# leohuang2013/pyannote-audio_speaker-diarization_cpp

Hardware: AMD Instinct MI355X
Metric: real-time factor (audio-sec/wall-sec), 1 h 16 kHz mono per GPU (higher is better)
Workload: dtype f32

## Files before the change

### pyannote-audio_speaker-diarization_cpp_amd/csrc/api.cpp

```cpp
#include "common.h"
#include "many_plan.h"
#include "wav_file.h"
#include "roster.h"
#include <algorithm>
#include <cmath>
#include <cstdlib>
#include <fstream>
#include <tuple>

static std::string g_create_err;

int seg_prec(const sd_ctx* c) { return c->seg_precision >= 0 ? c->seg_precision : (c->ecapa_precision != 0 ? 3 : 0); }

extern "C" const char* sd_create_error(void) { return g_create_err.c_str(); }
extern "C" const char* sd_last_error(const sd_ctx* c) { return c ? c->err.c_str() : "null context"; }

extern "C" sd_ctx* sd_create(const char* seg_path, const char* emb_path, int device)
{
    g_create_err.clear();
    int ndev = 0;
    if (hipGetDeviceCount(&ndev) != hipSuccess || ndev <= 0) { g_create_err = "no HIP device available (libsdhip has no CPU fallback)"; return nullptr; }
    if (device < 0 || device >= ndev) { g_create_err = "device id out of range"; return nullptr; }
    if (hipSetDevice(device) != hipSuccess) { g_create_err = "hipSetDevice failed"; return nullptr; }
    sd_ctx* c = new sd_ctx();
// ... 51 lines not shown
    }
    c->pending.clear();
}

extern "C" int sd_kernel_stats(const sd_ctx* cc, const char* kernel, double* total_ms, int64_t* launches, double* flops, double* bytes)
{
    sd_ctx* c = const_cast<sd_ctx*>(cc);
    if (!c || !kernel) return SD_ERR_ARG;
    (void)hipStreamSynchronize(c->stream);
    sd_flush_profile(c);
    auto it = c->stats.find(kernel);
    KernelStat s; if (it != c->stats.end()) s = it->second;
    if (total_ms) *total_ms = s.ms; if (launches) *launches = s.launches; if (flops) *flops = s.flops; if (bytes) *bytes = s.bytes;
    return SD_OK;
}
extern "C" int sd_debug_read_ws(sd_ctx* c, const char* name, int64_t offset, void* h_out, int64_t bytes)
{
    if (!c || !name || !h_out || offset < 0 || bytes < 0) return SD_ERR_ARG;
    auto it = c->ws.find(name);
    if (it == c->ws.end() || !it->second.p) SD_FAIL(c, SD_ERR_ARG, "no workspace named %s", name);
    if ((size_t)(offset + bytes) > it->second.cap) SD_FAIL(c, SD_ERR_ARG, "workspace %s holds %zu bytes", name, it->second.cap);
    HIPCHK(c, hipStreamSynchronize(c->stream));
    HIPCHK(c, hipMemcpy(h_out, (const char*)it->second.p + offset, (size_t)bytes, hipMemcpyDeviceToHost));
    return SD_OK;
}
extern "C" void sd_reset_stats(sd_ctx* c) { if (!c) return; (void)hipStreamSynchronize(c->stream); sd_flush_profile(c); c->stats.clear(); }
extern "C" int sd_stage_ms(const sd_ctx* c, double* ms4) { if (!c || !ms4) return SD_ERR_ARG; for (int i = 0; i < 4; ++i) ms4[i] = c->stage_ms[i]; return SD_OK; }
extern "C" int sd_set_option(sd_ctx* c, const char* key, int64_t v)
{
    if (!c || !key) return SD_ERR_ARG;
    std::string k(key);
    if (k == "emb_batch_items") { c->emb_batch_items = v; c->emb_batch_explicit = true; }
    else if (k == "seg_batch_chunks") c->seg_batch_chunks = v;
    else if (k == "ws_limit_mb") g_ws_limit.store(v > 0 ? (size_t)v << 20 : 0);
    else if (k == "emb_batch_default") { c->emb_batch_items = 3072; c->emb_batch_explicit = false; c->embed_calls = v; }
    else if (k == "linkage_wgs") c->linkage_wgs = v;
    else if (k == "linkage_threads") c->linkage_threads = v;
    else if (k == "linkage_kernel") c->linkage_kernel = v;
    else if (k == "linkage_tie_kernel") c->linkage_tie_kernel = v;
    else if (k == "linkage_zero_phase") c->linkage_zero_phase = v;
    else if (k == "linkage_force_heap") c->linkage_force_heap = v != 0;
    else if (k == "linkage_hx_wide") c->linkage_hx_wide = v != 0;
    else if (k == "linkage_prefetch") c->linkage_prefetch = v != 0;
    else if (k == "linkage_one_xcd") c->linkage_one_xcd = v;
    else if (k == "linkage_square") c->linkage_square = v;
    else if (k == "linkage_batch") { if (v != 0 && v != 1) SD_FAIL(c, SD_ERR_ARG, "linkage_batch must be 0 or 1"); c->linkage_batch = v; }
    else if (k == "linkage_batch_bytes") { if (v < 1) SD_FAIL(c, SD_ERR_ARG, "linkage_batch_bytes must be at least 1"); c->linkage_batch_bytes = v; }
    else if (k == "linkage_batch_threads") { if (v != 0 && v != 256 && v != 1024) SD_FAIL(c, SD_ERR_ARG, "linkage_batch_threads must be 0 (auto), 256 or 1024"); c->linkage_batch_threads = v; }
    else if (k == "skip_dead_rows") c->skip_dead_rows = v != 0;
    else if (k == "conv_h256") c->conv_h256 = v != 0;
    else if (k == "conv_glds") c->conv_glds = v != 0;
    else if (k == "conv_pp") c->conv_pp = v != 0;
    else if (k == "conv_glds_f32") c->conv_glds_f32 = v != 0;
    else if (k == "conv_mfma16") { if (v < 0 || v > 2) return SD_ERR_ARG; c->conv_mfma16 = (int)v; }
    else if (k == "conv_rot") { if (v < 0 || v > 3) return SD_ERR_ARG; c->conv_rot = (int)v; }
    else if (k == "conv_stagger") { if (v < 0 || v > 2) return SD_ERR_ARG; c->conv_stagger = (int)v; }
    else if (k == "conv_w256_f32") c->conv_w256_f32 = v != 0;
    else if (k == "conv_pn") c->conv_pn = (int)v;
    else if (k == "ecapa_ld_pad") { if (v < 0 || v > 1024 || ((int64_t)v & 7)) return SD_ERR_ARG; c->ecapa_ld_pad = (int)v; }
    else if (k == "seg_shared_conv0") c->seg_shared_conv0 = v != 0;
    else if (k == "seg_wide_ih") c->seg_wide_ih = v != 0;
    else if (k == "conv_w256_kmin") c->conv_w256_kmin = (int)v;
    else if (k == "conv_pn128") c->conv_pn128 = (int)v;
    else if (k == "seg_precision") { if (v != 0 && v != 3 && v != -1) SD_FAIL(c, SD_ERR_ARG, "seg_precision must be 0 (f32), 3 (split fp16 operands for the LSTM) or -1 (auto: 3 whenever ecapa_precision is not 0)"); c->seg_precision = (int)v; }
    else if (k == "ecapa_precision") { if (v < 0 || v > 3) SD_FAIL(c, SD_ERR_ARG, "ecapa_precision must be 0 (f32), 1 (fp16), 2 (fp16, hi + lo weight planes) or 3 (f32 tensors, split fp16 operands on the wide layers)");
                                        if (hipSetDevice(c->device) != hipSuccess) SD_FAIL(c, SD_ERR_HIP, "hipSetDevice failed");
                                        const int rcw = ensure_ecapa_mode_weights(c, (int)v); if (rcw) return rcw;
                                        c->ecapa_precision = (int)v; }
    else if (k == "ecapa_f16_hp") { if (v != 0 && v != 1 && v != 3) SD_FAIL(c, SD_ERR_ARG, "ecapa_f16_hp must be 0, 1 (MFA output in f32) or 3 (+ the attention branch)"); c->ecapa_f16_hp = (int)v; }
    else if (k == "ecapa_keep_cat") c->ecapa_keep_cat = v != 0;
    else if (k == "rank0_permille") c->rank0_permille = (int)v;
    else if (k == "virtual_world") c->virtual_world = (int)v;
    else if (k == "comm_timeout_ms") c->comm_timeout_ms = v;
    else if (k == "inject_fail_rank") c->inject_fail_rank = (int)v;
    else if (k == "constrained_assignment") c->constrained_assignment = v != 0;
    else if (k == "clustering_method") { if (v < SD_LINKAGE_SINGLE || v > SD_LINKAGE_WEIGHTED) SD_FAIL(c, SD_ERR_ARG, "clustering_method must be one of SD_LINKAGE_SINGLE (0) .. SD_LINKAGE_WEIGHTED (6)"); c->clustering_method = (int)v; }
    else if (k == "min_cluster_size") { if (v < 1 || v > 0x7fffffff) SD_FAIL(c, SD_ERR_ARG, "min_cluster_size must be at least 1"); c->min_cluster_size = (int)v; }
    else if (k == "max_num_embeddings") { if (v != -1 && v < 1) SD_FAIL(c, SD_ERR_ARG, "max_num_embeddings must be -1 (every train row) or at least 1"); c->max_num_embeddings = v; }
    else if (k == "clustering_seed") c->clustering_seed = v;
    else if (k == "num_clusters") c->num_clusters = (int)v;
    else if (k == "min_clusters") c->min_clusters = (int)v;
    else if (k == "max_clusters") c->max_clusters = (int)v;
    else if (k == "activity_hamming") { if (v != 0 && v != 1) SD_FAIL(c, SD_ERR_ARG, "activity_hamming must be 0 or 1"); c->activity_hamming = v != 0; }
    else if (k == "cut_group_bytes") { if (v < 1) SD_FAIL(c, SD_ERR_ARG, "cut_group_bytes must be at least 1"); c->cut_group_bytes = v; }
    else if (k == "profile") { c->profile = v != 0; c->profile_detail = v >= 2; }
    else SD_FAIL(c, SD_ERR_ARG, "unknown option %s", key);
    return SD_OK;
}

extern "C" int sd_set_option_f64(sd_ctx* c, const char* key, double v)
{
    if (!c || !key) return SD_ERR_ARG;
    std::string k(key);
    if (k == "clustering_threshold") { if (!(v >= 0.0 && v <= 2.0)) SD_FAIL(c, SD_ERR_ARG, "clustering_threshold must lie in [0, 2]"); c->clustering_threshold = v; }
    else if (k == "activity_onset") { if (!(v >= 0.0 && v <= 1.0)) SD_FAIL(c, SD_ERR_ARG, "activity_onset must lie in [0, 1]"); c->activity_onset = v; }
    else if (k == "activity_offset") { if (!(v >= 0.0 && v <= 1.0)) SD_FAIL(c, SD_ERR_ARG, "activity_offset must lie in [0, 1]"); c->activity_offset = v; }
    else if (k == "activity_min_duration_on") { if (!(v >= 0.0)) SD_FAIL(c, SD_ERR_ARG, "activity_min_duration_on must be >= 0"); c->activity_min_on = v; }
    else if (k == "activity_min_duration_off") { if (!(v >= 0.0)) SD_FAIL(c, SD_ERR_ARG, "activity_min_duration_off must be >= 0"); c->activity_min_off = v; }
    else if (k == "speaker_match_threshold") { if (!(v >= 0.0 && v <= 2.0)) SD_FAIL(c, SD_ERR_ARG, "speaker_match_threshold must lie in [0, 2]"); c->speaker_match_threshold = v; }
    else SD_FAIL(c, SD_ERR_ARG, "unknown real-valued option %s", key);
    return SD_OK;
}
extern "C" int sd_linkage_method_from_name(const char* name)
{
    static const char* const names[] = {"single", "complete", "average", "centroid", "median", "ward", "weighted"};
    if (!name) return -1;
// ... 462 lines not shown
```

### pyannote-audio_speaker-diarization_cpp_amd/csrc/common.h

```cpp
#pragma once
#include <hip/hip_runtime.h>
#include <atomic>
#include <chrono>
#include <cstdint>
#include <cstdio>
#include <cstring>
#include <map>
#include <set>
#include <string>
#include <functional>
#include <initializer_list>
#include <vector>
#include "../../include/sdhip_test.h"
#include "cluster_host.h"
#include "many_plan.h"

#define SD_T 501
#define SD_TP 501
#define SD_NBINS 201
#define SD_NMELS 80
#define SD_FEAT_LD 96

#define SD_WAV_PAD 512
struct DevWav {
// ... 14 lines not shown
    int reserve(size_t bytes) {
        if (bytes <= cap) return 0;
        const auto t0 = std::chrono::steady_clock::now();
        if (p) (void)hipFree(p);
        const auto t1 = std::chrono::steady_clock::now();
        p = nullptr; cap = 0;
        size_t want = bytes + (bytes >> 3) + 256;
        const size_t lim = g_ws_limit.load(std::memory_order_relaxed);
        if ((lim && bytes > lim) || hipMalloc(&p, want) != hipSuccess) { p = nullptr; (void)hipGetLastError(); return 1; }
        const auto t2 = std::chrono::steady_clock::now();
        g_ws_free_us += (long long)std::chrono::duration<double, std::micro>(t1 - t0).count();
        g_ws_alloc_us += (long long)std::chrono::duration<double, std::micro>(t2 - t1).count();
        g_ws_alloc_bytes += want; ++g_ws_allocs;
        cap = want; return 0;
    }
    void release() { if (p) (void)hipFree(p); p = nullptr; cap = 0; }
    template <class T> T* as() const { return (T*)p; }
};

struct ConvLayer {
    float* W = nullptr;
    void* W16 = nullptr;
    float* bias = nullptr;
    float* scale = nullptr;
    float* shift = nullptr;
    int Cin = 0, CinPad = 0, Cout = 0, KT = 1, dil = 1;
    int CinPad16 = 0;
    void* W16x = nullptr;
    float w16x_inv = 1.0f;
};

struct ConvArgs {
    const float* X; const float* X2; const float* W; float* Y;
    const void* W16;
    const float* bias; const float* scale; const float* shift; const float* item_bias; const float* R;
    int x_ld, x2_ld, y_ld, r_ld, ib_ld;
    int w_ld;
    int M;
    int TpIn, TpOut;
    int Tin, T;
    int Cin, Cout, KT, dil;
    int cin_real;
    int pad_mode;
    int act1, act2;
    int m_tiles, n_tiles;
    int sched;
    const int2* rowtab;
    int in_rows;
    int y_f32;
    int kt_real;
    int prec;
    const void* W16x;
    float acc_scale;
    int stagger;
};
#define ROWTAB_T(y) ((y) & 1023)
#define ROWTAB_LAST(y) (((y) >> 10) & 1023)
#define ROWTAB_ITEM(y) ((int)((unsigned)(y) >> 20))
#define ROWTAB_MAX_ITEMS 4095

struct EcapaWeights {
    bool loaded = false;
    float* mel_w = nullptr; int* mel_lo = nullptr; int* mel_cnt = nullptr; int* mel_off = nullptr; int mel_nnz = 0;
    float* window = nullptr;
    double* tw_cos = nullptr;
    double* tw_nsin = nullptr;
    ConvLayer block0;
    struct SERes { ConvLayer tdnn1, res[7], tdnn2, se1, se2; int dil; } blk[3];
    ConvLayer mfa, asp_tdnn_x, asp_tdnn_ms, asp_conv, fc;
    int C = 1024;
    std::vector<ConvLayer*> conv16;
    bool have16 = false, have16x = false;
};

struct SegWeights {
    bool loaded = false;
    float wn_w = 1, wn_b = 0;
    ConvLayer conv0, conv1, conv2;
    float* conv0_wsum = nullptr;
    float* in_w[3] = {nullptr, nullptr, nullptr};
    float* in_b[3] = {nullptr, nullptr, nullptr};
    ConvLayer lstm_ih[4];
    float* lstm_hh[4][2] = {};
    void* lstm_hh_x[4][2] = {};
    float lstm_hh_inv[4][2] = {};
    ConvLayer lin0, lin1;
    float* cls_w = nullptr; float* cls_b = nullptr;
};

struct StepStash {
    bool clustered = false;
    int64_t N = 0; int K = 0;
    std::vector<int> clusters, cluster_res, hard_pre;
    std::vector<double> X, Xn, soft;
    int64_t ar0 = 0, cr0 = 0, rows = 0, crow_all = 0, nact = 0;
    int64_t infer_items = 0;
};

struct JobResult { std::vector<double> conf, cen; std::vector<int64_t> cen_counts; int cen_K = 0, cen_d = 0; std::vector<int32_t> enrolled, hard, roster_ids; };

struct ManyJob { int status = SD_OK; JobResult res; };

struct sd_ctx {
    int device = 0;
    hipStream_t stream = nullptr;
    std::string err;
    EcapaWeights ew;
    SegWeights sw;
    std::vector<void*> owned;
    char* warena_cur = nullptr; size_t warena_left = 0;
    std::map<std::string, DevBuf> ws;
    std::set<std::string> rs_taps_filled;
    std::map<std::string, KernelStat> stats;
    bool profile = false;
    bool profile_detail = false;
    std::vector<std::tuple<std::string, hipEvent_t, hipEvent_t, double, double>> pending;
    double stage_ms[4] = {0, 0, 0, 0};
    int64_t emb_batch_items = 3072;
    bool emb_batch_explicit = false;
    int64_t embed_calls = 0;
    int64_t seg_batch_chunks = 4096;
    int num_clusters = -1, min_clusters = -1, max_clusters = -1;
    int ecapa_precision = 0;
    int seg_precision = -1;
    bool ecapa_keep_cat = false;
    int ecapa_f16_hp = 0;
    bool conv_w256_f32 = true;
    int conv_pn128 = 0;
    int ecapa_ld_pad = 0;
    bool seg_wide_ih = true;
    bool seg_shared_conv0 = true;
    int conv_w256_kmin = 0;
    int conv_pn = 0;
    bool conv_h256 = true;
    int conv_mfma16 = 1;
    int conv_rot = 3;
    int conv_stagger = 0;
    bool conv_glds_f32 = false;
    bool conv_pp = true;
    bool conv_glds = true;
    bool skip_dead_rows = true;
    int64_t linkage_wgs = -1;
    int64_t linkage_square = -1;
    int64_t linkage_one_xcd = 1;
    int64_t linkage_zero_phase = 1;
    int64_t linkage_tie_kernel = 1;
    int64_t linkage_prefetch = 0;
    bool linkage_hx_wide = false;
    bool linkage_force_heap = false;
    int64_t linkage_kernel = -1;
    int64_t linkage_threads = 0;
    int64_t linkage_batch = 0;
    int64_t linkage_batch_bytes = (int64_t)2 << 30;
    int64_t linkage_batch_threads = 0;
    std::vector<double> ahead_Z; int64_t ahead_N = -1;
    int num_cu = 256;
    bool constrained_assignment = false;
    int clustering_method = SD_LINKAGE_CENTROID;
    double clustering_threshold = (double)0.7153814381597874f;
    int min_cluster_size = 15;
    int64_t max_num_embeddings = -1;
    bool stream_intact = false;
    int64_t clustering_seed = 0;
    JobResult last;
    DevBuf enr_gal, enr_m2;
    std::vector<double> enr_host;
    int64_t enr_M = 0;
    int enr_d = 0;
    double speaker_match_threshold = (double)0.7153814381597874f * (double)0.7153814381597874f / 2;
    double activity_onset = 0.5, activity_offset = 0.5, activity_min_on = 0.0, activity_min_off = 0.0;
    bool activity_hamming = false;
    std::vector<double> last_activity;
    int64_t fe_bill_samples = -1, fe_bill_frames = 0;
    void* comm = nullptr;
    int rank = 0, world = 1;
    int virtual_world = 0;
    int64_t comm_timeout_ms = 600000;
    int64_t job_seq = 0;
    int inject_fail_rank = -1;
    int rank0_permille = -1;
    std::string dump_dir;
    int dump_level = 0;
    StepStash stash;
    std::string ws_failed;
    int fe_last_grid = 0;
    const char* last_conv_kernel = nullptr;
    const float* planted_scores = nullptr;
    const float* planted_emb = nullptr;
    int64_t planted_lo = 0, planted_n = 0;
    std::vector<ManyJob> many_jobs;
// ... 22 lines not shown
#define ENTER(ctx) do { if (!(ctx)) return SD_ERR_ARG; (ctx)->err.clear(); if (hipSetDevice((ctx)->device) != hipSuccess) SD_FAIL(ctx, SD_ERR_HIP, "hipSetDevice failed"); } while (0)
#define GRID1(n) dim3((unsigned)(((n) + 255) / 256)), dim3(256)
inline double now_ms() { return std::chrono::duration<double, std::milli>(std::chrono::steady_clock::now().time_since_epoch()).count(); }

struct ProfScope {
    sd_ctx* c; std::string name; hipEvent_t e0 = nullptr, e1 = nullptr; double flops, bytes;
    ProfScope(sd_ctx* ctx, const std::string& n, double fl = 0, double by = 0) : c(ctx), name(n), flops(fl), bytes(by) {
        if (c->profile) { (void)hipEventCreate(&e0); (void)hipEventCreate(&e1); (void)hipEventRecord(e0, c->stream); }
    }
    ~ProfScope() {
        if (c->profile) { (void)hipEventRecord(e1, c->stream); c->pending.emplace_back(name, e0, e1, flops, bytes); }
        else { KernelStat& s = c->stats[name]; s.launches++; s.flops += flops; s.bytes += bytes; }
    }
};
void sd_flush_profile(sd_ctx* c);

inline int conv_tiles_grid(const sd_ctx* c, ConvArgs& a, int tile_m, int tile_n, int wgs_per_cu)
{
    a.m_tiles = (a.M + tile_m - 1) / tile_m;
    a.n_tiles = (a.Cout + tile_n - 1) / tile_n;
    int g = (wgs_per_cu * c->num_cu / 8) * 8;
    if (g < 8) g = 8;
    const int lx_max = ((a.m_tiles + 7) / 8) * a.n_tiles;
    if (g / 8 > lx_max) g = lx_max * 8;
    return g;
}
struct ConvBill { double flops, bytes; };
inline ConvBill conv_bill(const ConvArgs& a, double rows, bool f16, int inputs = 1)
{
    const int cin = a.cin_real > 0 ? a.cin_real : a.Cin;
    const int kt_alg = a.kt_real > 0 ? a.kt_real : a.KT;
    return {2.0 * rows * a.Cout * cin * kt_alg, (f16 ? 2.0 : 4.0) * (rows * cin * inputs + rows * a.Cout + (double)a.Cout * cin * a.KT)};
}
inline bool conv_set_dyn_lds(const sd_ctx* c, std::atomic<unsigned>& mask, std::initializer_list<const void*> kernels, size_t lds_bytes)
{
    const unsigned dev_bit = 1u << (c->device & 31);
    if (mask.load(std::memory_order_acquire) & dev_bit) return true;
    for (const void* k : kernels)
        if (hipFuncSetAttribute(k, hipFuncAttributeMaxDynamicSharedMemorySize, (int)lds_bytes) != hipSuccess) { (void)hipGetLastError(); return false; }
    mask.fetch_or(dev_bit, std::memory_order_release);
    return true;
}
struct ConvProfWide {
    ProfScope all, prec, wide, caller;
    ConvProfWide(sd_ctx* c, const char* tag, const char* p, const ConvBill& b)
        : all(c, c->profile_detail ? std::string("conv_gemm:") + tag : std::string("conv_gemm"), b.flops, b.bytes),
          prec(c, std::string("conv_gemm_") + p, b.flops, b.bytes), wide(c, std::string("conv_w256_") + p, b.flops, b.bytes),
          caller(c, strcmp(tag, "lstm_ih") == 0 ? "conv_w256_seg" : "conv_w256_ecapa", b.flops, b.bytes) {}
};
int launch_conv_gemm(sd_ctx* c, const ConvArgs& a, const char* tag);
int launch_conv_gemm_h256(sd_ctx* c, const ConvArgs& a, const char* tag);
int launch_conv_gemm_g256(sd_ctx* c, const ConvArgs& a, const char* tag);
int launch_conv_gemm_pp(sd_ctx* c, const ConvArgs& a, const char* tag);
int seg_prec(const sd_ctx* c);
int launch_conv_narrow(sd_ctx* c, const ConvArgs& a, const char* tag);
struct PackTensor { std::vector<int64_t> dims; std::vector<float> data; };
typedef std::map<std::string, PackTensor> Pack;
int load_pack(const char* path, Pack& out, std::string& err);
int load_model_any(const char* path, int kind, Pack& out, std::string& err);
int build_ecapa_weights(sd_ctx* c, const Pack& p);
int build_seg_weights(sd_ctx* c, const Pack& p);
float lstm_whh_split(const float* whh , _Float16* planes );
void* weight_alloc(sd_ctx* c, size_t bytes);
int ensure_ecapa_mode_weights(sd_ctx* c, int ecapa_precision);
inline size_t conv_w16_bytes(const ConvLayer& L) { return (size_t)2 * L.KT * L.Cout * L.CinPad16 * 2; }
inline size_t conv_w16x_bytes(const ConvLayer& L) { return (size_t)2 * L.KT * L.Cout * L.CinPad * 2; }
int build_conv_w16(sd_ctx* c, ConvLayer& L, void* d);
int build_conv_w16x(sd_ctx* c, ConvLayer& L, void* d, unsigned* d_max);
int frontend_prepare(sd_ctx* c, const float* d_masks, int64_t items, int64_t first_item, float* d_wav_lens, int* d_nnorm, int* d_nvalid,
                     int* d_flags, bool compact, int* h_n_active, int* d_cidx, std::vector<int>* h_nvalid = nullptr);
int frontend_features(sd_ctx* c, const DevWav& w, int64_t first_item, int64_t run_items, bool compact, const int* d_nnorm,
                      const int* d_rowoff, float* d_feats , bool sig_mode = false);
int embed_signals_frames(sd_ctx* c, const float* h_wav_lens, int64_t B, std::vector<int>& nv, std::vector<int>& nn);
int frontend_prepare_signals(sd_ctx* c, int64_t items);
#define EC_SPACES 4
struct EcapaRowPlan {
    int64_t n = 0;
    std::vector<int> off[EC_SPACES];
    const int* d_off = nullptr;
};
int ecapa_need_rows(int nvalid, bool skip_dead_rows);
int ecapa_build_rowtab(sd_ctx* c, const int* d_off_out, int base_out, const int* d_off_in, int base_in, int64_t items, int2* d_rowtab);
int ecapa_rows_to_half(sd_ctx* c, const float* d_f32, void* d_f16, int64_t n4);
int ecapa_feats_to_half(sd_ctx* c, const float* d_f32, void* d_f16, int64_t rows);
int ecapa_scatter_emb(sd_ctx* c, const float* d_emb_c, const int* d_cidx, float* d_emb, int64_t items);
int launch_masked_mean(sd_ctx* c, bool f16, const void* x, int ld, const int* nvalid, const int* rowoff, int row_base, int64_t items, int64_t rows, float* out, int C);
int launch_se_apply(sd_ctx* c, bool f16, const void* t2, int t2_ld, const float* gate, const void* res, int res_ld, void* y, int y_ld, int C, int64_t rows,
                    const int2* rowtab, const int2* res_map, const int2* out_map);
int launch_asp_stats(sd_ctx* c, bool f16, const void* x, int ld, const int* nvalid, const int* rowoff, int row_base, int64_t items, int64_t rows, float* ms, int C);
int launch_asp_pool(sd_ctx* c, bool f16, const void* x, const float* logit, int ld, const int* nvalid, const int* rowoff, int row_base, int64_t items, int64_t rows,
                    float* pooled, int C);
int ecapa_row_plan(sd_ctx* c, const int* h_nvalid, int64_t n, EcapaRowPlan& plan, int* d_off );
int run_ecapa(sd_ctx* c, const float* d_feats, const int* d_nvalid , const EcapaRowPlan& plan, int64_t a0, int64_t a1, float* d_emb );
std::vector<int64_t> ecapa_plan_batches(const EcapaRowPlan& plan, int64_t cap_rows, bool balance);
int64_t ecapa_round_items(int64_t nb);
int ecapa_run_items(sd_ctx* c, const float* d_feats, const int* d_nvalid, const EcapaRowPlan& plan, int64_t nb, bool balance, float* d_emb);
int run_embed(sd_ctx* c, const DevWav& w, const float* d_masks, int64_t items, int64_t first_item, float* d_emb);
int run_segment(sd_ctx* c, const DevWav& w, int64_t chunk_lo, int64_t chunk_hi, float* d_seg);
int run_segment_rows(sd_ctx* c, const DevWav& rows, int T, float* d_seg, int* frames);
int launch_chunk_norm(sd_ctx* c, const float* d_wav, int64_t origin, int64_t first_chunk, int64_t hop, int L, int64_t chunks, float w, float b, float* xn);
int launch_chunk_stats(sd_ctx* c, const float* d_wav, int64_t origin, int64_t first_chunk, int L, int64_t chunks, float w, float b, float2* st);
int launch_pool_norm(sd_ctx* c, int stage, const float* in, int64_t chunks, int Lc, const float* gw, const float* gb, float* out,
                     const float2* cst, const float* wsum, int chunk_rows);
int launch_lstm_rec(sd_ctx* c, const float* G, const float* whh_f, const float* whh_b, const void* whx_f, const void* whx_b, float inv_f, float inv_b,
                    float* H, int64_t B, int F);
int launch_classifier(sd_ctx* c, const float* y, const float* W, const float* bias, float* seg, int64_t chunks, int F);
// ... 62 lines not shown
```

### pyannote-audio_speaker-diarization_cpp_amd/csrc/conv_gemm.hip

```cpp
#include "conv_dev.h"
#include <type_traits>

#define BM 128
#define BN 128
#define BK 32
#define LDP 36
#define SD_CONV_SCHED_DEFAULT 3

template <bool HAS_X2, int PR>
__global__ __launch_bounds__(256, 2) void k_conv_gemm(ConvArgs a)
{
    constexpr bool F16 = PR == 1, X3 = PR == 3;
    __shared__ __attribute__((aligned(16))) float As[2][BM * LDP];
    __shared__ __attribute__((aligned(16))) float Bs[2][BN * LDP];

    ConvSched sch;
    int q0;
    if (!sch.init(a, a.sched >= 100 ? a.sched - 100 : 8 , q0)) return;
    const int wl = sch.wl, wpx = sch.wpx;

    const int tid = threadIdx.x;
    const int lane = tid & 63, wid = tid >> 6;
    const int wr = wid >> 1, wc = wid & 1;
    const int c4 = tid & 7, r0 = tid >> 3;
// ... 391 lines not shown
        acc = __builtin_amdgcn_mfma_f32_32x32x2f32(av.x, bv.x, acc, 0, 0, 0);
        acc = __builtin_amdgcn_mfma_f32_32x32x2f32(av.y, bv.y, acc, 0, 0, 0);
        acc = __builtin_amdgcn_mfma_f32_32x32x2f32(av.z, bv.z, acc, 0, 0, 0);
        acc = __builtin_amdgcn_mfma_f32_32x32x2f32(av.w, bv.w, acc, 0, 0, 0);
    }
    if (w > 0) {
#pragma unroll
        for (int r = 0; r < 16; ++r) part[w - 1][r][lane] = acc[r];
    }
    __syncthreads();
    if (w != 0) return;
    const int co = n0 + li;
    const bool col_ok = co < a.Cout;
    const float cb = (a.bias && col_ok) ? a.bias[co] : 0.0f;
    const float cs = (a.scale && col_ok) ? a.scale[co] : 1.0f, ch = (a.scale && col_ok) ? a.shift[co] : 0.0f;
    const float slope = conv_act_slope(a.act1);
#pragma unroll
    for (int r = 0; r < 16; ++r) {
        float v = ((acc[r] + part[0][r][lane]) + part[1][r][lane]) + part[2][r][lane];
        v += cb;
        v = v > 0.0f ? v : v * slope;
        v = v * cs + ch;
        if (a.act2 == 1) v = tanhf(v);
        else if (a.act2 == 2) v = 1.0f / (1.0f + expf(-v));
        const int g = m0 + (r & 3) + 8 * (r >> 2) + 4 * lh;
        if (g < a.M && col_ok) a.Y[(size_t)g * a.y_ld + co] = v;
    }
}

int launch_conv_gemm(sd_ctx* c, const ConvArgs& in, const char* tag)
{
    ConvArgs a = in;
    if (a.w_ld <= 0) a.w_ld = a.Cin;
    const bool f16 = a.prec == 1;
    if (f16 && !a.W16) SD_FAIL(c, SD_ERR_ARG, "conv_gemm(%s): fp16 mode without fp16 weights", tag);
    if (a.Cin % (f16 ? 64 : BK) != 0) SD_FAIL(c, SD_ERR_ARG, "conv_gemm(%s): Cin=%d not a multiple of %d", tag, a.Cin, f16 ? 64 : BK);
    if (a.M <= 0) return SD_OK;
    if (f16 && c->conv_h256 && c->conv_pp) { const int r = launch_conv_gemm_pp(c, a, tag); if (r != 1) return r; }
    if ((f16 && c->conv_h256 && c->conv_glds) || (!f16 && a.prec == 0 && c->conv_w256_f32 && c->conv_glds_f32)) { const int r = launch_conv_gemm_g256(c, a, tag); if (r != 1) return r; }
    if ((f16 && c->conv_h256) || (!f16 && c->conv_w256_f32) || a.prec == 3) { const int r = launch_conv_gemm_h256(c, a, tag); if (r != 1) return r; }
    const bool x3 = a.prec == 3 && a.W16x != nullptr;
    if (a.prec == 3 && !x3) a.prec = 0;
    if (x3) a.w_ld = 2 * a.Cin;
    if (a.prec == 0 && a.KT == 1 && a.M <= SD_SKINNY_MAX_ROWS && a.TpIn == a.M && a.TpOut == a.M && a.T == a.M && a.Tin == a.M && !a.X2 && !a.item_bias && !a.R && !a.rowtab &&
        (a.x_ld & 3) == 0 && (a.w_ld & 3) == 0) {
        const int cinr = a.cin_real > 0 ? a.cin_real : a.Cin;
        ProfScope ps(c, c->profile_detail ? std::string("skinny_gemm:") + tag : std::string("skinny_gemm"), 2.0 * a.M * a.Cout * cinr,
                     4.0 * ((double)a.M * cinr + (double)a.M * a.Cout + (double)a.Cout * cinr));
        c->last_conv_kernel = "skinny";
        hipLaunchKernelGGL(k_skinny_gemm, dim3((a.M + 31) / 32, (a.Cout + 31) / 32), dim3(256), 0, c->stream, a);
        KCHECK(c);
        return SD_OK;
    }
    a.sched = c->conv_pn128 > 0 ? 100 + c->conv_pn128 : SD_CONV_SCHED_DEFAULT;
    a.stagger = c->conv_stagger;
    const int grid = conv_tiles_grid(c, a, BM, BN, 2);
    const double rows = a.rowtab ? (double)a.M
                                 : (double)(a.M / a.TpOut) * a.T + (double)((a.M % a.TpOut) < a.T ? (a.M % a.TpOut) : a.T);
    const ConvBill bill = conv_bill(a, rows, f16, a.X2 ? 2 : 1);
    ProfScope ps(c, c->profile_detail ? std::string("conv_gemm:") + tag : std::string("conv_gemm"), bill.flops, bill.bytes);
    ProfScope ps16(c, f16 ? "conv_gemm_f16" : x3 ? "conv_gemm_x3" : "conv_gemm_f32", bill.flops, bill.bytes);
    c->last_conv_kernel = f16 ? (a.X2 ? "gemm128_f16_x2" : "gemm128_f16") : x3 ? (a.X2 ? "gemm128_x3_x2" : "gemm128_x3") : (a.X2 ? "gemm128_f32_x2" : "gemm128_f32");
    if (f16) {
        if (a.X2) hipLaunchKernelGGL((k_conv_gemm<true, 1>), dim3(grid), dim3(256), 0, c->stream, a);
        else hipLaunchKernelGGL((k_conv_gemm<false, 1>), dim3(grid), dim3(256), 0, c->stream, a);
    } else if (x3) {
        if (a.X2) hipLaunchKernelGGL((k_conv_gemm<true, 3>), dim3(grid), dim3(256), 0, c->stream, a);
        else hipLaunchKernelGGL((k_conv_gemm<false, 3>), dim3(grid), dim3(256), 0, c->stream, a);
    } else if (a.X2) hipLaunchKernelGGL((k_conv_gemm<true, 0>), dim3(grid), dim3(256), 0, c->stream, a);
    else hipLaunchKernelGGL((k_conv_gemm<false, 0>), dim3(grid), dim3(256), 0, c->stream, a);
    KCHECK(c);
    return SD_OK;
}

__global__ void k_fill_rand(float* p, int64_t n, unsigned seed)
{
    int64_t i = (int64_t)blockIdx.x * blockDim.x + threadIdx.x;
    if (i >= n) return;
    unsigned x = (unsigned)i * 2654435761u + seed;
    x ^= x >> 15; x *= 2246822519u; x ^= x >> 13;
    p[i] = ((float)(x & 0xffffff) / 8388608.0f - 1.0f) * 0.5f;
}

extern "C" int sd_bench_conv(sd_ctx* c, int64_t items, int Tp, int T, int Cin, int Cout, int KT, int dil, int has_x2, int dbg, int reps, double* ms_per_launch)
{
    if (!c || !ms_per_launch || items <= 0 || Cin % BK) return SD_ERR_ARG;
    c->err.clear();
    if (hipSetDevice(c->device) != hipSuccess) return SD_ERR_HIP;
    const int64_t M = items * Tp;
    if (dbg < 0 || dbg % 10 != 0) SD_FAIL(c, SD_ERR_ARG, "sd_bench_conv: ablation %d: the ablation builds of k_conv_gemm are retired", dbg % 10);
    const int pad = (dbg / 100) * 32;
    dbg %= 100;
    const int xld = Cin + pad, wld = Cin + pad, yld = Cout + pad;
    WS(c, float, X, "bc_X", M * xld);
    WS(c, float, X2, "bc_X2", has_x2 ? M * xld : 16);
    WS(c, float, W, "bc_W", (int64_t)KT * Cout * wld);
    WS(c, float, Y, "bc_Y", M * yld);
    WS(c, float, B, "bc_B", 3 * Cout);
    hipLaunchKernelGGL(k_fill_rand, dim3((unsigned)((M * xld + 255) / 256)), dim3(256), 0, c->stream, X, M * xld, 1u);
    if (has_x2) hipLaunchKernelGGL(k_fill_rand, dim3((unsigned)((M * xld + 255) / 256)), dim3(256), 0, c->stream, X2, M * xld, 2u);
    hipLaunchKernelGGL(k_fill_rand, dim3((unsigned)(((int64_t)KT * Cout * wld + 255) / 256)), dim3(256), 0, c->stream, W, (int64_t)KT * Cout * wld, 3u);
    hipLaunchKernelGGL(k_fill_rand, dim3((unsigned)((3 * Cout + 255) / 256)), dim3(256), 0, c->stream, B, (int64_t)3 * Cout, 4u);
    ConvArgs a; memset(&a, 0, sizeof(a));
    a.X = X; a.x_ld = xld; a.X2 = has_x2 ? X2 : nullptr; a.x2_ld = xld; a.W = W; a.w_ld = wld; a.Y = Y; a.y_ld = yld;
    a.bias = B; a.scale = B + Cout; a.shift = B + 2 * Cout; a.act1 = 1;
    a.M = (int)M; a.TpIn = a.TpOut = Tp; a.Tin = a.T = T; a.Cin = Cin; a.Cout = Cout; a.KT = KT; a.dil = dil; a.pad_mode = 0;
// ... 17 lines not shown
```

### pyannote-audio_speaker-diarization_cpp_amd/csrc/ecapa.hip

```cpp
#include "common.h"
#include <algorithm>

template <class T> __global__ void k_masked_mean(const T* __restrict__ x, int ld, const int* __restrict__ nvalid, const int* __restrict__ rowoff, int row_base,
                              float* __restrict__ out, int C)
{
    const int item = blockIdx.y, ch = blockIdx.x * blockDim.x + threadIdx.x;
    if (ch >= C) return;
    const int nv = nvalid[item];
    const T* p = x + (size_t)(rowoff[item] - row_base) * ld + ch;
    float s0 = 0, s1 = 0, s2 = 0, s3 = 0;
    int t = 0;
    for (; t + 3 < nv; t += 4) { s0 += (float)p[(size_t)t * ld]; s1 += (float)p[(size_t)(t + 1) * ld]; s2 += (float)p[(size_t)(t + 2) * ld]; s3 += (float)p[(size_t)(t + 3) * ld]; }
    for (; t < nv; ++t) s0 += (float)p[(size_t)t * ld];
    out[(size_t)item * C + ch] = ((s0 + s1) + (s2 + s3)) / (float)nv;
}

template <class T> struct Vec4;
template <> struct Vec4<float> { typedef float4 type; };
template <> struct Vec4<_Float16> { typedef _Float16 type __attribute__((ext_vector_type(4))); };
template <class T> __device__ __forceinline__ float4 ld4(const T* p)
{
    if constexpr (sizeof(T) == 4) return *(const float4*)p;
    else { const typename Vec4<_Float16>::type h = *(const typename Vec4<_Float16>::type*)p; return make_float4((float)h[0], (float)h[1], (float)h[2], (float)h[3]); }
}
// ... 215 lines not shown
    const float* d_feats = d_feats_all + (size_t)rbase[0] * SD_FEAT_LD;
    const int* d_nvalid = d_nvalid_all + a0;
    float* d_emb = d_emb_all + (size_t)a0 * SD_EMB_DIM;
    const int64_t M = R[0], MN = R[3];
    if (M > 0x7fffffff / 2) SD_FAIL(c, SD_ERR_ARG, "ecapa batch too large");
    WS(c, T, x0, "ec_x0", M * LD);
    const int LDT = 2 * C - C / 8 + c->ecapa_ld_pad;
    WS(c, T, tr, "ec_tr", M * LDT);
    WS(c, T, t2, "ec_t2", R[1] * LD);
    WS(c, T, cat, "ec_cat", R[1] * LD3);
    WS(c, T, mfa, "ec_mfa", MN * LD3);
    WS(c, T, hid, "ec_hid", MN * 128);
    WS(c, float, se_s, "ec_se_s", items * C);
    WS(c, float, se_h, "ec_se_h", items * 128);
    WS(c, float, se_g, "ec_se_g", items * C);
    WS(c, float, ms, "ec_ms", items * 2 * C3);
    WS(c, float, ib, "ec_ib", items * 128);
    WS(c, float, pooled, "ec_pooled", items * 2 * C3);
    int rc;
    const bool f16 = sizeof(T) == 2;
    int2* tabs[EC_SPACES][EC_SPACES] = {};
    auto tab = [&](int so, int si) -> int2* {
        if (tabs[so][si]) return tabs[so][si];
        char key[32]; snprintf(key, sizeof(key), "ec_rowtab_%d%d", so, si);
        int2* p = ws_get<int2>(c, key, (size_t)R[so] + 128);
        if (!p) return nullptr;
        if (ecapa_build_rowtab(c, ro[so], rbase[so], ro[si], rbase[si], items, p)) return nullptr;
        tabs[so][si] = p;
        return p;
    };
#define TAB(var, so, si) int2* var = tab(so, si); if (!var) SD_FAIL(c, SD_ERR_HIP, "hipMalloc of a row table failed")

    const void* f_in = d_feats; int f_ld = SD_FEAT_LD;
    if (sizeof(T) == 2) {
        WS(c, _Float16, fh, "ec_feats16", M * 128);
        if ((rc = ecapa_feats_to_half(c, d_feats, fh, M))) return rc;
        f_in = fh; f_ld = 128;
    }
    { TAB(t00, 0, 0); ConvArgs a = conv_args(E.block0, f_in, f_ld, x0, LD, M, true, P); a.act1 = 1; a.rowtab = t00; if ((rc = launch_conv_gemm(c, a, "block0"))) return rc; }

    for (int b = 0; b < 3; ++b) {
        const auto& B = E.blk[b];
        const int cs = b, os = b + 1, is = b == 0 ? 0 : 1;
        const int64_t Mc = R[cs], Mo = R[os];
        const T* xin = (b == 0) ? x0 : cat + (size_t)(b - 1) * C;
        const int xin_ld = (b == 0) ? LD : LD3;
        TAB(t_in, cs, is); TAB(t_cc, cs, cs); TAB(t_oc, os, cs);
        { ConvArgs a = conv_args(B.tdnn1, xin, xin_ld, tr, LDT, Mc, true, P); a.act1 = 1; a.rowtab = t_in; a.in_rows = (int)R[is]; if ((rc = launch_conv_gemm(c, a, "tdnn1"))) return rc; }
        const int S = C / 8;
        for (int i = 1; i < 8; ++i) {
            ConvArgs a = conv_args(B.res[i - 1], tr + (i - 1) * S, LDT, tr + C + (i - 1) * S, LDT, Mc, true, P);
            a.act1 = 1;
            if (i >= 2) { a.X2 = (const float*)(tr + C + (i - 2) * S); a.x2_ld = LDT; }
            a.rowtab = t_cc;
            if ((rc = launch_conv_gemm(c, a, "res2net"))) return rc;
        }
        { ConvArgs a = conv_args(B.tdnn2, tr + C - S, LDT, t2, LD, Mo, true, P); a.act1 = 1; a.rowtab = t_oc; a.in_rows = (int)Mc; if ((rc = launch_conv_gemm(c, a, "tdnn2"))) return rc; }
        if ((rc = launch_masked_mean(c, f16, t2, LD, d_nvalid, ro[os], rbase[os], items, Mo, se_s, C))) return rc;
        { ConvArgs a = conv_args(B.se1, se_s, C, se_h, 128, items, false); a.act1 = 1; if ((rc = launch_conv_gemm(c, a, "se1"))) return rc; }
        { ConvArgs a = conv_args(B.se2, se_h, 128, se_g, C, items, false); a.act2 = 2; if ((rc = launch_conv_gemm(c, a, "se2"))) return rc; }
        {
            const int2* res_map = nullptr; const int2* out_map = nullptr;
            if (os != is) { TAB(m, os, is); res_map = m; }
            if (os != 1) { TAB(m, os, 1); out_map = m; }
            if ((rc = launch_se_apply(c, f16, t2, LD, se_g, xin, xin_ld, cat + (size_t)b * C, LD3, C, Mo, t_oc, res_map, out_map))) return rc;
        }
    }
    TAB(t31, 3, 1); TAB(t33, 3, 3);
    const int hp = sizeof(T) == 2 ? c->ecapa_f16_hp : 0;
    float* mfa32 = nullptr;
    if (hp & 1) { WS(c, float, m32, "ec_mfa32", MN * LD3); mfa32 = m32; }
    {
        ConvArgs a = conv_args(E.mfa, cat, LD3, mfa32 ? (void*)mfa32 : (void*)mfa, LD3, MN, true, P);
        a.act1 = 1; a.rowtab = t31; a.in_rows = (int)R[1]; a.y_f32 = mfa32 ? 1 : 0;
        if ((rc = launch_conv_gemm(c, a, "mfa"))) return rc;
    }
    if (mfa32 && !(hp & 2)) {
        if ((rc = ecapa_rows_to_half(c, mfa32, mfa, MN * LD3 / 4))) return rc;
    }
    const void* pool_x = mfa32 ? (const void*)mfa32 : (const void*)mfa;
    const bool pool_f16 = f16 && !mfa32;
    if ((rc = launch_asp_stats(c, pool_f16, pool_x, LD3, d_nvalid, ro[3], rbase[3], items, MN, ms, C3))) return rc;
    { ConvArgs a = conv_args(E.asp_tdnn_ms, ms, 2 * C3, ib, 128, items, false); if ((rc = launch_conv_gemm(c, a, "asp_ms"))) return rc; }
    float* logits;
    if (sizeof(T) == 2 || c->ecapa_keep_cat) { WS(c, float, lg, "ec_logits", MN * LD3); logits = lg; } else logits = (float*)cat;
    if (hp & 2) {
        WS(c, float, hid32, "ec_hid32", MN * 128);
        { ConvArgs a = conv_args(E.asp_tdnn_x, mfa32, LD3, hid32, 128, MN, true, 0); a.act1 = 1; a.act2 = 1; a.item_bias = ib; a.ib_ld = 128; a.rowtab = t33; if ((rc = launch_conv_gemm(c, a, "asp_tdnn"))) return rc; }
        { ConvArgs a = conv_args(E.asp_conv, hid32, 128, logits, LD3, MN, true, 0); a.rowtab = t33; if ((rc = launch_conv_gemm(c, a, "asp_conv"))) return rc; }
    } else {
        { ConvArgs a = conv_args(E.asp_tdnn_x, mfa, LD3, hid, 128, MN, true, P); a.act1 = 1; a.act2 = 1; a.item_bias = ib; a.ib_ld = 128; a.rowtab = t33; if ((rc = launch_conv_gemm(c, a, "asp_tdnn"))) return rc; }
        { ConvArgs a = conv_args(E.asp_conv, hid, 128, logits, LD3, MN, true, P); a.rowtab = t33; a.y_f32 = 1; if ((rc = launch_conv_gemm(c, a, "asp_conv"))) return rc; }
    }
    if ((rc = launch_asp_pool(c, pool_f16, pool_x, logits, LD3, d_nvalid, ro[3], rbase[3], items, MN, pooled, C3))) return rc;
    { ConvArgs a = conv_args(E.fc, pooled, 2 * C3, d_emb, SD_EMB_DIM, items, false); if ((rc = launch_conv_gemm(c, a, "fc"))) return rc; }
    return SD_OK;
}

__global__ void k_flag_nonfinite(const float* e, int64_t n, int* flag)
{
    const int64_t i = (int64_t)blockIdx.x * blockDim.x + threadIdx.x;
    if (i < n && !isfinite(e[i])) *flag = 1;
}

int run_ecapa(sd_ctx* c, const float* d_feats, const int* d_nvalid, const EcapaRowPlan& plan, int64_t a0, int64_t a1, float* d_emb)
{
    if (c->ecapa_precision == 1 || c->ecapa_precision == 2) return run_ecapa_t<_Float16>(c, d_feats, d_nvalid, plan, a0, a1, d_emb);
// ... 175 lines not shown
```

Baseline: 2968.

## Add persistent panel kernel for f32 Res2Net dilated convolutions

```diff
diff --git a/pyannote-audio_speaker-diarization_cpp_amd/csrc/api.cpp b/pyannote-audio_speaker-diarization_cpp_amd/csrc/api.cpp
--- a/pyannote-audio_speaker-diarization_cpp_amd/csrc/api.cpp
+++ b/pyannote-audio_speaker-diarization_cpp_amd/csrc/api.cpp
@@ -127,6 +127,7 @@
     else if (k == "conv_glds") c->conv_glds = v != 0;
     else if (k == "conv_pp") c->conv_pp = v != 0;
     else if (k == "conv_glds_f32") c->conv_glds_f32 = v != 0;
+    else if (k == "conv_res2_panel") c->conv_res2_panel = v != 0;
     else if (k == "conv_mfma16") { if (v < 0 || v > 2) return SD_ERR_ARG; c->conv_mfma16 = (int)v; }
     else if (k == "conv_rot") { if (v < 0 || v > 3) return SD_ERR_ARG; c->conv_rot = (int)v; }
     else if (k == "conv_stagger") { if (v < 0 || v > 2) return SD_ERR_ARG; c->conv_stagger = (int)v; }
diff --git a/pyannote-audio_speaker-diarization_cpp_amd/csrc/common.h b/pyannote-audio_speaker-diarization_cpp_amd/csrc/common.h
--- a/pyannote-audio_speaker-diarization_cpp_amd/csrc/common.h
+++ b/pyannote-audio_speaker-diarization_cpp_amd/csrc/common.h
@@ -90,6 +90,7 @@
     int prec;
     const void* W16x;
     float acc_scale;
+    int same_space;
     int stagger;
 };
 #define ROWTAB_T(y) ((y) & 1023)
@@ -174,6 +175,7 @@
     int conv_mfma16 = 1;
     int conv_rot = 3;
     int conv_stagger = 0;
+    bool conv_res2_panel = true;
     bool conv_glds_f32 = false;
     bool conv_pp = true;
     bool conv_glds = true;
@@ -302,6 +304,7 @@
 int launch_conv_gemm_h256(sd_ctx* c, const ConvArgs& a, const char* tag);
 int launch_conv_gemm_g256(sd_ctx* c, const ConvArgs& a, const char* tag);
 int launch_conv_gemm_pp(sd_ctx* c, const ConvArgs& a, const char* tag);
+int launch_conv_res2_panel(sd_ctx* c, const ConvArgs& a, const char* tag);
 int seg_prec(const sd_ctx* c);
 int launch_conv_narrow(sd_ctx* c, const ConvArgs& a, const char* tag);
 struct PackTensor { std::vector<int64_t> dims; std::vector<float> data; };
diff --git a/pyannote-audio_speaker-diarization_cpp_amd/csrc/conv_gemm.hip b/pyannote-audio_speaker-diarization_cpp_amd/csrc/conv_gemm.hip
--- a/pyannote-audio_speaker-diarization_cpp_amd/csrc/conv_gemm.hip
+++ b/pyannote-audio_speaker-diarization_cpp_amd/csrc/conv_gemm.hip
@@ -467,6 +467,7 @@
         KCHECK(c);
         return SD_OK;
     }
+    { const int r = launch_conv_res2_panel(c, a, tag); if (r != 1) return r; }
     a.sched = c->conv_pn128 > 0 ? 100 + c->conv_pn128 : SD_CONV_SCHED_DEFAULT;
     a.stagger = c->conv_stagger;
     const int grid = conv_tiles_grid(c, a, BM, BN, 2);
diff --git a/pyannote-audio_speaker-diarization_cpp_amd/csrc/conv_res2.hip b/pyannote-audio_speaker-diarization_cpp_amd/csrc/conv_res2.hip
--- /dev/null
+++ b/pyannote-audio_speaker-diarization_cpp_amd/csrc/conv_res2.hip
@@ -0,0 +1,191 @@
+#include "conv_dev.h"
+
+#define RP_BM 128
+#define RP_HALO 4
+#define RP_ROWS (RP_BM + 2 * RP_HALO)
+#define RP_LD 132
+#define RP_WLD 36
+#define RP_PARTS ((RP_ROWS * 32 + 511) / 512)
+#define RP_LDS_BYTES ((RP_ROWS * RP_LD + 2 * 128 * RP_WLD) * 4)
+
+static std::atomic<unsigned> g_attr_res2{0};
+
+template <bool HAS_X2>
+__global__ __launch_bounds__(512, 1) void k_conv_res2_panel(ConvArgs a)
+{
+    extern __shared__ __attribute__((aligned(16))) float lds[];
+    float* const Ps = lds;
+    float* const Ws = lds + RP_ROWS * RP_LD;
+
+    const int G = gridDim.x;
+    int tile = blockIdx.x;
+    if (tile >= a.m_tiles) return;
+    const int tid = threadIdx.x, lane = tid & 63, wid = tid >> 6;
+    const int wr = wid >> 1, wc = wid & 1, li = lane & 31, lh = lane >> 5;
+    const int d = a.dil;
+    const int in_rows = a.M;
+    const int prow = tid >> 5, pch = tid & 31;
+    const int wrow = tid >> 3, wch = tid & 7;
+
+    auto panel_rsrc = [&](const float* X, int ld, int m0, bool live) {
+        int lo = m0 - d; if (lo < 0) lo = 0;
+        int hi = m0 + RP_BM + d; if (hi > in_rows) hi = in_rows;
+        const int rows = live && hi > lo ? hi - lo : 0;
+        return conv_rsrc(X + (live ? (size_t)lo * ld : 0), (size_t)rows * ld * 4);
+    };
+    const unsigned voA0 = (unsigned)(prow * a.x_ld + pch * 4) * 4u, stA = (unsigned)a.x_ld * 64u;
+    const unsigned voX0 = HAS_X2 ? (unsigned)(prow * a.x2_ld + pch * 4) * 4u : 0u, stX = HAS_X2 ? (unsigned)a.x2_ld * 64u : 0u;
+    f4u pa[RP_PARTS], px[2];
+    auto pstore = [&]() {
+#pragma unroll
+        for (int p = 0; p < RP_PARTS; ++p)
+            if (prow + 16 * p < RP_ROWS) *(float4*)&Ps[(prow + 16 * p) * RP_LD + pch * 4] = make_float4(pa[p][0], pa[p][1], pa[p][2], pa[p][3]);
+    };
+
+    const __amdgpu_buffer_rsrc_t rB = conv_rsrc(a.W, (size_t)3 * 128 * a.w_ld * 4);
+    const unsigned voB0 = (unsigned)(wrow * a.w_ld + wch * 4) * 4u, stB = (unsigned)a.w_ld * 256u;
+    f4u rb[2];
+    auto wload = [&](int s) {
+        const unsigned so = (unsigned)((s >> 2) * 128 * a.w_ld + (s & 3) * 32) * 4u;
+        rb[0] = __builtin_bit_cast(f4u, __builtin_amdgcn_raw_buffer_load_b128(rB, voB0, so, 0));
+        rb[1] = __builtin_bit_cast(f4u, __builtin_amdgcn_raw_buffer_load_b128(rB, voB0 + stB, so, 0));
+    };
+    auto wstore = [&](int buf) {
+#pragma unroll
+        for (int p = 0; p < 2; ++p) *(float4*)&Ws[buf * 128 * RP_WLD + (wrow + 64 * p) * RP_WLD + wch * 4] = make_float4(rb[p][0], rb[p][1], rb[p][2], rb[p][3]);
+    };
+
+    int poff[3];
+    auto set_rows = [&](int2 e, int m0) {
+        const int t = ROWTAB_T(e.y), last = ROWTAB_LAST(e.y);
+#pragma unroll
+        for (int kk = 0; kk < 3; ++kk) {
+            int pr = e.x + conv_src_frame(t, kk, 3, 1, d, a.Tin, last) - (m0 - d);
+            pr = pr < 0 ? 0 : (pr > RP_ROWS - 1 ? RP_ROWS - 1 : pr);
+            poff[kk] = pr * RP_LD + lh * 16;
+        }
+    };
+    auto tab_entry = [&](int m0) { const int g = m0 + wr * 32 + li; return a.rowtab[g < a.M ? g : a.M - 1]; };
+
+    f32x16 acc[2];
+#pragma unroll
+    for (int j = 0; j < 2; ++j)
+#pragma unroll
+        for (int r = 0; r < 16; ++r) acc[j][r] = 0.0f;
+    const int boff = (wc * 64 + li) * RP_WLD + lh * 16;
+    float4 fa[2], fb[2][2];
+    auto lfrag = [&](int s, int qq, int set) {
+        const float* Ab = Ps + poff[s >> 2] + (s & 3) * 32 + qq * 4;
+        const float* Bb = Ws + (s & 1) * 128 * RP_WLD + boff + qq * 4;
+        fa[set] = *(const float4*)Ab;
+        fb[set][0] = *(const float4*)Bb;
+        fb[set][1] = *(const float4*)(Bb + 32 * RP_WLD);
+    };
+    auto mma8 = [&](int set) {
+        const float av[4] = {fa[set].x, fa[set].y, fa[set].z, fa[set].w};
+        const float bv0[4] = {fb[set][0].x, fb[set][0].y, fb[set][0].z, fb[set][0].w}, bv1[4] = {fb[set][1].x, fb[set][1].y, fb[set][1].z, fb[set][1].w};
+#pragma unroll
+        for (int e = 0; e < 4; ++e) {
+            acc[0] = __builtin_amdgcn_mfma_f32_32x32x2f32(av[e], bv0[e], acc[0], 0, 0, 0);
+            acc[1] = __builtin_amdgcn_mfma_f32_32x32x2f32(av[e], bv1[e], acc[1], 0, 0, 0);
+        }
+    };
+
+    int m0 = tile * RP_BM;
+    {
+        const int shift = m0 < d ? d - m0 : 0;
+        const __amdgpu_buffer_rsrc_t rA = panel_rsrc(a.X, a.x_ld, m0, true), rX = panel_rsrc(HAS_X2 ? a.X2 : a.X, HAS_X2 ? a.x2_ld : a.x_ld, m0, true);
+#pragma unroll
+        for (int p = 0; p < RP_PARTS; ++p) {
+            const bool ok = prow + 16 * p >= shift;
+            pa[p] = __builtin_bit_cast(f4u, __builtin_amdgcn_raw_buffer_load_b128(rA, ok ? voA0 + p * stA - (unsigned)shift * a.x_ld * 4u : 0x80000000u, 0, 0));
+            if (HAS_X2) pa[p] += __builtin_bit_cast(f4u, __builtin_amdgcn_raw_buffer_load_b128(rX, ok ? voX0 + p * stX - (unsigned)shift * a.x2_ld * 4u : 0x80000000u, 0, 0));
+        }
+        wload(0);
+        set_rows(tab_entry(m0), m0);
+        pstore();
+        wstore(0);
+    }
+    __syncthreads();
+    lfrag(0, 0, 0);
+
+    const float slope = conv_act_slope(a.act1);
+    const unsigned ybytes = (unsigned)a.y_ld * 4u;
+    float cb_[2], cs_[2], ch_[2];
+#pragma unroll
+    for (int j = 0; j < 2; ++j) conv_col_params(a, wc * 64 + j * 32 + li, cb_[j], cs_[j], ch_[j]);
+
+    while (true) {
+        const int ntile = tile + G;
+        const bool has_next = ntile < a.m_tiles;
+        const int m0n = ntile * RP_BM;
+        const __amdgpu_buffer_rsrc_t rA = panel_rsrc(a.X, a.x_ld, m0n, has_next), rX = panel_rsrc(HAS_X2 ? a.X2 : a.X, HAS_X2 ? a.x2_ld : a.x_ld, m0n, has_next);
+        const int2 en = tab_entry(has_next ? m0n : m0);
+
+#pragma unroll
+        for (int s = 0; s < 12; ++s) {
+            lfrag(s, 1, 1);
+            wload((s + 1) % 12);
+            if (s < RP_PARTS) {
+                pa[s] = __builtin_bit_cast(f4u, __builtin_amdgcn_raw_buffer_load_b128(rA, voA0 + s * stA, 0, 0));
+                if (HAS_X2) px[s & 1] = __builtin_bit_cast(f4u, __builtin_amdgcn_raw_buffer_load_b128(rX, voX0 + s * stX, 0, 0));
+            }
+            mma8(0);
+            CONV_MFMA_PAIR(0x100, 3);
+            CONV_MFMA_PAIR(0x020, (s < RP_PARTS ? (HAS_X2 ? 4 : 3) : 2));
+            __builtin_amdgcn_sched_barrier(0);
+            lfrag(s, 2, 0);
+            mma8(1);
+            CONV_MFMA_PAIR(0x100, 3);
+            __builtin_amdgcn_sched_barrier(0);
+            lfrag(s, 3, 1);
+            if (HAS_X2 && s >= 1 && s <= RP_PARTS) pa[s - 1] += px[(s - 1) & 1];
+            wstore((s + 1) & 1);
+            mma8(0);
+            CONV_MFMA_PAIR(0x100, 3);
+            CONV_MFMA_PAIR(0x200, 2);
+            __builtin_amdgcn_sched_barrier(0);
+            __syncthreads();
+            if (s < 11) {
+                lfrag(s + 1, 0, 0);
+                mma8(1);
+                CONV_MFMA_PAIR(0x100, 3);
+                __builtin_amdgcn_sched_barrier(0);
+            } else {
+                pstore();
+                mma8(1);
+                CONV_MFMA_PAIR(0x200, 7);
+                __builtin_amdgcn_sched_barrier(0);
+                __syncthreads();
+                set_rows(en, m0n);
+                lfrag(0, 0, 0);
+            }
+        }
+
+        const __amdgpu_buffer_rsrc_t rY = conv_out_rsrc((char*)a.Y + (size_t)m0 * ybytes, a.M - m0, RP_BM, ybytes);
+#pragma unroll
+        for (int j = 0; j < 2; ++j)
+            conv_store_rows<false>(acc[j], rY, (unsigned)(wr * 32 + 4 * lh) * ybytes + (unsigned)(wc * 64 + j * 32 + li) * 4u, ybytes, false, 1.0f, cb_[j], slope, cs_[j], ch_[j]);
+        if (!has_next) break;
+        tile = ntile; m0 = m0n;
+    }
+}
+
+int launch_conv_res2_panel(sd_ctx* c, const ConvArgs& in, const char* tag)
+{
+    ConvArgs a = in;
+    if (!c->conv_res2_panel || a.prec != 0 || a.KT != 3 || a.kt_real != 0 || a.Cin != 128 || a.Cout != 128 || a.dil < 1 || a.dil > RP_HALO || a.pad_mode != 0 ||
+        a.item_bias || a.R || a.act2 != 0 || ((a.x_ld | a.y_ld | a.w_ld) & 3) || (a.X2 && (a.x2_ld & 3)) || a.M < 2048 ||
+        !a.rowtab || !a.same_space || (a.in_rows != 0 && a.in_rows != a.M)) return 1;
+    if (!conv_set_dyn_lds(c, g_attr_res2, {(const void*)k_conv_res2_panel<false>, (const void*)k_conv_res2_panel<true>}, RP_LDS_BYTES)) return 1;
+    a.m_tiles = (a.M + RP_BM - 1) / RP_BM; a.n_tiles = 1;
+    const int grid = a.m_tiles < c->num_cu ? a.m_tiles : c->num_cu;
+    const ConvBill bill = conv_bill(a, (double)a.M, false, a.X2 ? 2 : 1);
+    ProfScope ps(c, c->profile_detail ? std::string("conv_gemm:") + tag : std::string("conv_gemm"), bill.flops, bill.bytes);
+    ProfScope ps32(c, "conv_gemm_f32", bill.flops, bill.bytes);
+    c->last_conv_kernel = a.X2 ? "res2_panel_f32_x2" : "res2_panel_f32";
+    if (a.X2) hipLaunchKernelGGL((k_conv_res2_panel<true>), dim3(grid), dim3(512), RP_LDS_BYTES, c->stream, a);
+    else hipLaunchKernelGGL((k_conv_res2_panel<false>), dim3(grid), dim3(512), RP_LDS_BYTES, c->stream, a);
+    KCHECK(c);
+    return SD_OK;
+}
diff --git a/pyannote-audio_speaker-diarization_cpp_amd/csrc/ecapa.hip b/pyannote-audio_speaker-diarization_cpp_amd/csrc/ecapa.hip
--- a/pyannote-audio_speaker-diarization_cpp_amd/csrc/ecapa.hip
+++ b/pyannote-audio_speaker-diarization_cpp_amd/csrc/ecapa.hip
@@ -291,7 +291,7 @@
             ConvArgs a = conv_args(B.res[i - 1], tr + (i - 1) * S, LDT, tr + C + (i - 1) * S, LDT, Mc, true, P);
             a.act1 = 1;
             if (i >= 2) { a.X2 = (const float*)(tr + C + (i - 2) * S); a.x2_ld = LDT; }
-            a.rowtab = t_cc;
+            a.rowtab = t_cc; a.same_space = 1;
             if ((rc = launch_conv_gemm(c, a, "res2net"))) return rc;
         }
         { ConvArgs a = conv_args(B.tdnn2, tr + C - S, LDT, t2, LD, Mo, true, P); a.act1 = 1; a.rowtab = t_oc; a.in_rows = (int)Mc; if ((rc = launch_conv_gemm(c, a, "tdnn2"))) return rc; }
```

After: 2995 (median of 6 runs). About the same (+0.9%).
